# knights-lab/UTree

Hardware: AMD Instinct MI355X
Metric: reads classified/sec, 8 GB L2 CTR, 150 bp reads (higher is better)
Workload: dtype u64; 1 GPU; configs[1]: 1.22e+09-node synthetic L2 CTR (k=32, 21844 labels, image 40.8 GiB, fine_bits=8), 1152000000 x 150 bp reads per GPU (72 steps x 16000000-read batches, 41 distinct batches resident in HBM), RC=0

## Files before the change

utree_amd/csrc/dev_image.c:

```c
#define _FILE_OFFSET_BITS 64
#define _GNU_SOURCE
#define __HIP_PLATFORM_AMD__ 1
#include <hip/hip_runtime_api.h>
#include <fcntl.h>
#include <math.h>
#include <stddef.h>
#include <stdio.h>
#include <stdlib.h>
#include <string.h>
#include <unistd.h>
#include "ctr_host.h"
#include "dev_image.h"

#define HIPCHK(x) do { hipError_t e_ = (x); if (e_ != hipSuccess) { utree_dev_set_hip_error((int)e_, #x); rc = e_ == hipErrorOutOfMemory ? UTREE_E_NOMEM : UTREE_E_HIP; goto fail; } } while (0)
#define KCHK(x) do { int e_ = (x); if (e_ != 0) { utree_dev_set_hip_error(e_, #x); rc = e_ == (int)hipErrorOutOfMemory ? UTREE_E_NOMEM : UTREE_E_HIP; goto fail; } } while (0)

static __thread char g_hip_msg[256];
void utree_dev_set_hip_error(int err, const char *what) {
    snprintf(g_hip_msg, sizeof g_hip_msg, "%s (%d) in %s", hipGetErrorString((hipError_t)err), err, what);
    if (getenv("UTREE_DEBUG")) fprintf(stderr, "[utree_amd] HIP error: %s\n", g_hip_msg);
}
const char *utree_last_hip_error(void) { return g_hip_msg; }
void utree_set_error_text(const char *msg) { snprintf(g_hip_msg, sizeof g_hip_msg, "%s", msg); }

// ... 592 lines not shown
    info->lane_pass = utk_lanes_image_ok(&d->kimg) != 0;
    info->bucket_bytes = 8u * d->hdr.bucket_words;
    info->strand_views = (d->hdr.flags & UTREE_F_STRAND_VIEWS) ? 1u : 0u;
    if (d->hdr.flags & UTREE_F_DIRECT) info->bucket_bytes = 0;
    info->overflow_chains = (d->hdr.flags & UTREE_F_OVF_CHAINS) ? 1u : 0u;
    info->pad0 = 0;
    info->overflow_bytes = (d->hdr.flags & UTREE_F_DIRECT) ? 0 : d->hdr.n_min * d->hdr.rec_words * 8;
    return UTREE_OK;
}

#define LONG_BLOCKS_PER_CU 8

static uint32_t mid_limit(void) {
    static uint32_t v = 0;
    if (!v) {
        const char *e = getenv("UTREE_MID_LIMIT");
        v = UTREE_MID_DEFAULT;
        if (e && atoi(e) >= (int)UTREE_SHORT2_CAP && atoi(e) <= (int)UTREE_MID_CAP) v = (uint32_t)atoi(e);
    }
    return v;
}

static int lanes_enabled(void) { const char *e = getenv("UTREE_LANE_PASS"); return !(e && e[0] == '0'); }

static void ring_lock(utree_dev *d) { while (__atomic_test_and_set(&d->ring_busy, __ATOMIC_ACQUIRE)) ; }
static void ring_unlock(utree_dev *d) { __atomic_clear(&d->ring_busy, __ATOMIC_RELEASE); }

static void ring_collect(utree_dev *d) {
    if (!d->lanes_ring) return;
    ring_lock(d);
    for (unsigned i = 0; i < 64; ++i) {
        const unsigned long long left = d->lanes_ring[2 * i], err = d->lanes_ring[2 * i + 1];
        if (left == ~0ull || err == ~0ull) continue;
        d->lanes_ring[2 * i] = ~0ull; d->lanes_ring[2 * i + 1] = ~0ull;
        d->ring_inflight[i] = 0;
        if (err && !d->dev_error) d->dev_error = err;
        if (timing_on()) fprintf(stderr, "[utree_amd] batch report: %llu of %u reads left by the lane pass, error word %llu\n", left, d->lanes_ring_reads[i], err);
        if (d->lanes_ring_reads[i]) {
            if (left * 4 <= d->lanes_ring_reads[i]) { unsigned long long n = 0, l = 0; for (unsigned w = 0; w < UTREE_LANES_WINDOW; ++w) { n += d->win_reads[w]; l += d->win_left[w]; }
                if (n >= (1u << 18) && l * 4 > n) { memset(d->win_left, 0, sizeof d->win_left); memset(d->win_reads, 0, sizeof d->win_reads); } }
            const unsigned w = d->win_next++ % UTREE_LANES_WINDOW;
            d->win_left[w] = left; d->win_reads[w] = d->lanes_ring_reads[i];
        }
        d->lanes_ring_reads[i] = 0;
    }
    ring_unlock(d);
// ... 63 lines not shown
    char *b = (char *)ws;
    w->cursors = (unsigned long long *)(b + off); off = align_up(off + UTREE_CURSOR_BYTES, 256);
    const uint64_t waves_per_cu = 32 + 20 + 5 * 12;
    w->tally_cap = ((do_rc ? 2 : 1) * total_bases + (uint64_t)n_reads) * 9 / 8 + (uint64_t)d->n_cu * waves_per_cu * UTREE_TALLY_CHUNK + 4096;
    { const char *e = getenv("UTREE_TEST_TALLY_CAP"); if (e && atoll(e) > 0 && (uint64_t)atoll(e) < w->tally_cap) w->tally_cap = (uint64_t)atoll(e); }
    { uint64_t room = w->tally_cap; if (room < UTREE_TALLY_CHUNK) room = UTREE_TALLY_CHUNK; if (room < d->hdr.n_labels) room = d->hdr.n_labels;
      w->tally = (uint64_t *)(b + off); off = align_up(off + room * 8, 256); }
    w->long_list = (uint32_t *)(b + off); off = align_up(off + (uint64_t)n_reads * 4, 256);
    w->mid_list = (uint32_t *)(b + off); off = align_up(off + (uint64_t)n_reads * 4, 256);
    uint64_t max_total = do_rc ? 2 * (uint64_t)max_len + 1 : max_len;
    w->long_blocks = 0; w->hist = NULL; w->touch = NULL;
    w->short_cap = max_total > UTREE_SHORT_CAP ? UTREE_SHORT2_CAP : UTREE_SHORT_CAP;
    w->mid_reads = max_total > w->short_cap;
    w->mid_limit = mid_limit();
    const int lanes_img = utk_lanes_image_ok(&d->kimg);
    if (max_total > w->mid_limit || (lanes_img && max_len > utk_lanes_max_len(&d->kimg))) {
        w->long_blocks = (uint32_t)d->n_cu * LONG_BLOCKS_PER_CU;
        if (w->long_blocks > n_reads) w->long_blocks = n_reads;
        w->hist = (uint32_t *)(b + off); off = align_up(off + (uint64_t)w->long_blocks * d->hdr.n_labels * 4, 256);
        w->touch = (uint32_t *)(b + off); off = align_up(off + (uint64_t)w->long_blocks * ((d->hdr.n_labels + 31) / 32) * 4, 256);
    }
    w->pieces = NULL; w->ltab_rank = w->ltab_cnt = w->lflag = w->long_left = NULL; w->n_long_cap = 0; w->ltally_base = 0;
    w->cls_list = NULL; w->cls_stride = 0; w->n_pieces_cap = 0;
    if (lanes_img && max_len > UTREE_LANES_CAP) {
        w->cls_stride = (n_reads + 63u) & ~63u;
        w->cls_list = (uint32_t *)(b + off); off = align_up(off + (uint64_t)5 * w->cls_stride * 4, 256);
    }
    if (lanes_img && w->long_blocks) {
        uint64_t cap = total_bases / lanes_long_min(d, do_rc) + 1;
        if (cap > n_reads) cap = n_reads;
        const uint64_t piece_windows = 16ull * (UTREE_LANES_CAP - 4 * d->hdr.W + 1);
        const uint64_t n_pieces = total_bases / piece_windows + cap + 1;
        w->n_long_cap = (uint32_t)cap;
        w->n_pieces_cap = n_pieces;
        w->pieces = (uint64_t *)(b + off); off = align_up(off + n_pieces * 8, 256);
        w->ltab_rank = (uint32_t *)(b + off); off = align_up(off + cap * UTREE_LONG_SLOTS * 4, 256);
        w->ltab_cnt = (uint32_t *)(b + off); off = align_up(off + cap * UTREE_LONG_SLOTS * 4, 256);
        w->lflag = (uint32_t *)(b + off); off = align_up(off + cap * 4, 256);
        w->long_left = (uint32_t *)(b + off); off = align_up(off + cap * 4, 256);
        w->ltally_base = (uint64_t)((uint64_t *)(b + off) - w->tally); off = align_up(off + cap * UTREE_LONG_SLOTS * 8, 256);
        { const char *e = getenv("UTREE_TEST_LONG_CAP"); if (e && atoll(e) > 0 && (uint64_t)atoll(e) < w->n_long_cap) w->n_long_cap = (uint32_t)atoll(e); }
        { const char *e = getenv("UTREE_TEST_PIECES_CAP"); if (e && atoll(e) > 0 && (uint64_t)atoll(e) < w->n_pieces_cap) w->n_pieces_cap = (uint64_t)atoll(e); }
    }
    *bytes = (size_t)off;
}

// ... 23 lines not shown
                                 const uint8_t *d_text, uint64_t text_bytes, const uint32_t *d_name_off, const uint32_t *d_name_len) {
    int rc = UTREE_OK;
    if (!d || !d_out || (!d_workspace && n_reads)) return UTREE_E_ARG;
    if (!n_reads) return UTREE_OK;
    if (!d_bases || !d_off || !d_len) return UTREE_E_ARG;
    hipStream_t st = (hipStream_t)stream;
    utk_workspace w; size_t need;
    carve(d, d_workspace, n_reads, total_bases, max_len, do_rc, &w, &need);
    if (workspace_bytes < need) return UTREE_E_ARG;
    HIPCHK(hipSetDevice(d->device));
    HIPCHK(hipMemsetAsync(w.cursors, 0, UTREE_CURSOR_BYTES, st));
    if (w.long_blocks) {
        HIPCHK(hipMemsetAsync(w.hist, 0, (size_t)w.long_blocks * d->hdr.n_labels * 4, st));
        HIPCHK(hipMemsetAsync(w.touch, 0, (size_t)w.long_blocks * ((d->hdr.n_labels + 31) / 32) * 4, st));
    }
    hipEvent_t e0 = NULL, e1 = NULL;
    int tslot = -1;
    if (__atomic_load_n(&d->timing_on, __ATOMIC_ACQUIRE)) {
        tslot = __atomic_fetch_add(&d->n_claimed, 1, __ATOMIC_RELAXED);
        if (tslot >= 0 && tslot < UTREE_MAX_PENDING && 2 * tslot + 1 < d->n_events) { e0 = d->events[2 * tslot]; e1 = d->events[2 * tslot + 1]; }
        else tslot = -1;
    }
    ring_collect(d);
    const int lanes = lanes_enabled() && utk_lanes_image_ok(&d->kimg) && lanes_worth(d);
    if (lanes) {
        const int mixed = max_len > UTREE_LANES_CAP;
        d->last_long = w.long_blocks != 0; d->last_mid = 0; d->last_rc = do_rc; d->last_short_cap = w.short_cap;
        d->last_lanes = utk_lanes_segs(&d->kimg, max_len); d->last_mixed = mixed; d->last_pieces = w.long_blocks != 0;
        if (e0 && !w.long_blocks) HIPCHK(hipEventRecord(e0, st));
        if (!mixed) KCHK(utk_classify_lanes(&d->kimg, d_bases, d_off, d_len, n_reads, max_len, do_rc, d_out, &w, d->n_cu, st));
        else KCHK(utk_classify_lanes_mixed(&d->kimg, d_bases, d_off, d_len, n_reads, max_len, do_rc, d_out, &w, d->n_cu, st));
        if (w.long_blocks) {
            if (e0) HIPCHK(hipEventRecord(e0, st));
            HIPCHK(hipMemsetAsync(w.ltab_rank, 0xFF, (size_t)w.n_long_cap * UTREE_LONG_SLOTS * 4, st));
            HIPCHK(hipMemsetAsync(w.ltab_cnt, 0, (size_t)w.n_long_cap * UTREE_LONG_SLOTS * 4, st));
            HIPCHK(hipMemsetAsync(w.lflag, 0, (size_t)w.n_long_cap * 4, st));
            KCHK(utk_classify_long_pieces(&d->kimg, d_bases, d_off, d_len, do_rc, d_out, &w, d->n_cu, st));
            utk_workspace wl = w;
            wl.long_list = w.long_left;
            wl.long_blocks = w.long_blocks >= 8 ? w.long_blocks / 8 : 1;
            KCHK(utk_classify_long(&d->kimg, d_bases, d_off, d_len, do_rc, d_out, &wl, d->n_cu, st));
            if (e0) { HIPCHK(hipEventRecord(e1, st)); d->recorded[tslot] = 1; }
        }
        KCHK(utk_classify_listed(&d->kimg, d_bases, d_off, d_len, n_reads, max_len, do_rc, d_out, &w, d->n_cu, st));
        if (e0 && !w.long_blocks) { HIPCHK(hipEventRecord(e1, st)); d->recorded[tslot] = 1; }
    } else {
// ... 107 lines not shown
```

utree_amd/csrc/kernels.hip:

```cpp
#include <hip/hip_runtime.h>
#include <stdint.h>
#include <stdio.h>
#include <string.h>
#include "device_common.hpp"
#include "wave_common.hpp"

using namespace utk;

namespace {

#ifdef UTREE_PHASE_TIMERS
__device__ unsigned long long g_phase[16];
struct PhaseT { unsigned long long t, acc[12]; };
#define PH_DECL PhaseT ph_; ph_.t = __builtin_readcyclecounter(); for (int q_ = 0; q_ < 12; ++q_) ph_.acc[q_] = 0;
#define TICKP(ph, i) do { const unsigned long long n_ = __builtin_readcyclecounter(); (ph).acc[i] += n_ - (ph).t; (ph).t = n_; } while (0)
#define TICK(i) TICKP(ph_, i)
#define PH_ARG , PhaseT &ph_
#define PH_PASS , ph_
#define PH_WAITVM asm volatile("s_waitcnt vmcnt(0)" ::: "memory")
#else
#define PH_DECL
#define TICK(i)
#define PH_ARG
#define PH_PASS
// ... 249 lines not shown
        any = any || (nz & low_bytes(total > 4u * g ? total - 4u * g : 0u)) != 0u;
        const uint32_t nib = (nz * 0x00204081u) >> 28;
        const uint32_t nib_next = (uint32_t)__builtin_amdgcn_update_dpp(0, (int)nib, 0x101, 0xF, 0xF, true);
        uint32_t code = g2 ^ ((g2 >> 1) & 0x01010101u);
        code ^= rm & 0x03030303u;
        const uint32_t packed = (code * 0x40100401u) >> 24;
        if (g < ngroups) {
            sb[g ^ 3u] = (uint8_t)packed;
            if (!(lane & 1u)) sbadb[g >> 1] = (uint8_t)(nib | (nib_next << 4));
        }
    }
    return __ballot(any) != 0ull;
}

constexpr int SHORT_CAP = UTREE_SHORT_CAP;
constexpr int SHORT2_CAP = UTREE_SHORT2_CAP;
constexpr int MID_CAP = UTREE_MID_CAP;
constexpr int WAVES_PER_BLOCK = 4;
constexpr uint32_t WORK_GRAB = 32;
constexpr uint32_t TALLY_CHUNK = UTREE_TALLY_CHUNK;
constexpr uint32_t TALLY_DIRECT = UTREE_TALLY_CHUNK / 16;
constexpr int32_t CUT_PENDING = -3;
constexpr int32_t RANK_PENDING = -4;

constexpr int SHORT_MIN_WAVES = 8;
template <int W, int I, bool EXC, typename OFF, int CAP, bool LISTED, int RCMODE = 2>
__global__ __launch_bounds__(256, CAP > SHORT2_CAP ? (I == 2 ? 4 : 3) : (I == 2 ? SHORT_MIN_WAVES : 5))
void classify_short_k(utk_image im, const uint8_t *__restrict__ bases, const uint64_t *__restrict__ off,
                      const uint32_t *__restrict__ len, uint32_t n_reads, int do_rc_arg, utree_result *__restrict__ out,
                      utk_workspace ws) {
    if constexpr (LISTED) { if (!ws.cursors[UTREE_CUR_MID]) return; }
    const int do_rc = RCMODE == 2 ? do_rc_arg : RCMODE;
    constexpr uint32_t K = 4 * W;
    constexpr int NCH = CAP / 64, NWORDS = CAP / 16 + 6;
    __shared__ uint32_t s_words[WAVES_PER_BLOCK][NWORDS + 2];
    __shared__ uint64_t s_bad[WAVES_PER_BLOCK][NCH + 2];
    using HIT = typename std::conditional<I == 2, uint16_t, uint32_t>::type;
    __shared__ HIT s_hits[WAVES_PER_BLOCK][CAP];
    constexpr uint32_t TILE = CAP <= SHORT_CAP ? 256u : KEY_TILE;
    __shared__ uint64_t s_keys[WAVES_PER_BLOCK][TILE + 128];
    __shared__ uint64_t s_reg[256];
    constexpr bool PREFETCH = CAP <= SHORT2_CAP;
    static_assert(PREFETCH || sizeof(HIT) * CAP >= 4 * (RawBuf<CAP>::DW + 4), "raw bytes must fit the hit list");
    __shared__ uint32_t s_raw[PREFETCH ? WAVES_PER_BLOCK : 1][PREFETCH ? RawBuf<CAP>::DW + 4 : 1];
    stage_regions(im, s_reg);
    const RegionLds rg = {s_reg, (uint64_t)(uintptr_t)im.table, im.bucket_words == 16u ? 7u : 6u};
// ... 353 lines not shown
            before = idx ? ((uint32_t)(x1 >> (8 * idx - 8)) & 0xFFu) : prevlast;
            return;
        }
        prevlast = (uint32_t)(x1 >> 56); base += 8;
    }
}

struct VRec { uint64_t w[4]; };
__device__ __forceinline__ VRec vrec(const uint64_t *vt, uint32_t rank) {
    typedef unsigned long long u64x2 __attribute__((ext_vector_type(2)));
    const u64x2 *p = (const u64x2 *)(vt + (size_t)rank * 4);
    const u64x2 a = p[0], b = p[1];
    VRec v; v.w[0] = a.x; v.w[1] = a.y; v.w[2] = b.x; v.w[3] = b.y;
    return v;
}
__device__ __forceinline__ uint32_t v_pid(const VRec &v, uint32_t t) { return (uint32_t)((t < 4 ? v.w[0] : v.w[1]) >> (16u * (t & 3u))) & 0xFFFFu; }
__device__ __forceinline__ uint32_t v_end(const VRec &v, uint32_t t) { return (uint32_t)(v.w[2] >> (8u * t)) & 0xFFu; }
__device__ __forceinline__ bool v_exists(const VRec &v, uint32_t t) { return ((uint32_t)v.w[3] >> t) & 1u; }
__device__ __forceinline__ bool v_more(const VRec &v, uint32_t t) { return ((uint32_t)v.w[3] >> (8u + t)) & 1u; }
__device__ __forceinline__ bool v_us(const VRec &v, uint32_t t) { return ((uint32_t)v.w[3] >> (16u + t)) & 1u; }
__device__ __forceinline__ uint32_t v_len(const VRec &v) { return (uint32_t)(v.w[3] >> 32) & 0xFFu; }
__device__ __forceinline__ uint32_t v_ix(const VRec &v) { return (uint32_t)(v.w[3] >> 48); }

__device__ __forceinline__ void vote_table(const utk_image &im, utree_result *out_r, const uint64_t *T, uint32_t F, uint32_t uix) {
    const uint64_t *vt = im.vote_tab;
    const char *blob = im.label_blob;
    const uint32_t *loff = im.label_off;
    constexpr uint32_t NONE = 0xFFFFFFFFu;
    uint32_t cutoff = cut_of(F);
    uint32_t st = 0, ed = uix, dv = NONE, t = 0, orun = F, sl, ol;
    uint32_t ix_last, n_last, len_last;
    for (;;) {
        const uint64_t t_st = T[st];
        VRec pv = vrec(vt, (uint32_t)t_st);
        const uint64_t t_ed = ed - 1u == st ? t_st : T[ed - 1u];
        const VRec lv = ed - 1u == st ? pv : vrec(vt, (uint32_t)t_ed);
        {
            const uint64_t d0 = pv.w[0] ^ lv.w[0], d1 = pv.w[1] ^ lv.w[1];
            const uint32_t same = d0 ? (uint32_t)__builtin_ctzll(d0) >> 4 : 4u + (d1 ? (uint32_t)__builtin_ctzll(d1) >> 4 : 4u);
            const uint32_t both = ((uint32_t)(pv.w[3] & lv.w[3]) >> 8) & 0xFFu;
            const uint32_t semis = (uint32_t)__builtin_ctz(~both);
            const uint32_t L = same < semis ? same : semis;
            if (L > t) { dv = v_end(pv, L - 1u); t = L; }
        }
        uint32_t run = (uint32_t)(t_st >> 32), td = dv, c1 = run, rp = (uint32_t)t_st;
        bool td_is_end = false;
        bool stopped = false;
        for (uint32_t z = st + 1; z < ed; ++z) {
            const bool is_last = z == ed - 1u;
            const uint64_t tz = is_last ? t_ed : T[z];
            const uint32_t nz = (uint32_t)(tz >> 32), rc = (uint32_t)tz;
            const VRec cv = is_last ? lv : vrec(vt, rc);
            bool aside = false, stop = false;
            if (t >= 8u || !v_exists(pv, t) || (dv == NONE && v_end(pv, 0) == 0u && !v_more(pv, 0))) aside = true;
            else {
                uint32_t a, b, before;
                bool known = true;
                if (v_exists(cv, t) && v_pid(cv, t) == v_pid(pv, t)) {
                    td = v_end(pv, t); td_is_end = true;
                    a = v_more(pv, t) ? ';' : 0u; b = v_more(cv, t) ? ';' : 0u; before = v_us(pv, t) ? '_' : 'x';
                } else if (v_us(pv, t) || !v_exists(cv, t)) {
                    pair_scan(blob + loff[rp], blob + loff[rc], dv + 1u, td, a, b, before);
                    td_is_end = td == v_end(pv, t);
                } else { a = 'a'; b = 'b'; before = 'x'; known = false; }
                if (a == b) run += nz;
                else if ((!a && b == ';') || ((a == ';' || !a) && before == '_')) aside = true;
                else if (run >= cutoff) {
                    ed = z; stop = true;
                    if (!known) {
                        pair_scan(blob + loff[rp], blob + loff[rc], dv + 1u, td, a, b, before);
                        td_is_end = td == v_end(pv, t);
                    }
                } else { run = nz; st = z; }
// ... 5 lines not shown
            }
            if (stop) { stopped = true; break; }
            pv = cv; c1 = nz; rp = rc;
        }
        ix_last = stopped ? v_ix(pv) : v_ix(lv);
        n_last = stopped ? c1 : (uint32_t)(t_ed >> 32);
        len_last = stopped ? v_len(pv) : v_len(lv);
        sl = run; ol = orun;
        if (run < cutoff) break;
        if (st + 1 >= ed) {
            if (n_last >= cutoff) dv = 0xFFFFFFFEu;
            break;
        }
        orun = run; cutoff = cut_of(run);
        if (td != dv) { dv = td; if (td_is_end) ++t; }
    }
    int32_t cut;
    if (dv == NONE) cut = -1;
    else if (dv == 0xFFFFFFFEu) cut = -2;
    else cut = (int32_t)(dv < len_last ? dv : len_last);
    store_result(out_r, ix_last, cut, F, uix, sl, ol);
}

__global__ __launch_bounds__(256) void vote_table_k(utk_image im, utree_result *__restrict__ out, utk_workspace ws, uint32_t n_reads) {
    __shared__ uint32_t s_n[2][4];
    __shared__ uint16_t s_who[256];
    const uint32_t tid = threadIdx.x, wv = tid >> 6, lane = tid & 63u;
    const uint32_t r0 = blockIdx.x * blockDim.x + tid;
    uint32_t cls = 2;
    if (r0 < n_reads) {
        const uint32_t *res = (const uint32_t *)&out[r0];
        const int32_t cut = (int32_t)res[1];
        if (cut == RANK_PENDING) {
            uint32_t *o = (uint32_t *)&out[r0];
            o[0] = im.rank2ix[res[0]]; o[1] = (uint32_t)-2;
        } else if (cut == CUT_PENDING) cls = res[3] == 2u ? 0u : 1u;
    }
    const uint64_t m0 = __builtin_amdgcn_ballot_w64(cls == 0u), m1 = __builtin_amdgcn_ballot_w64(cls == 1u);
    s_who[tid] = 0xFFFFu;
    if (lane == 0) { s_n[0][wv] = (uint32_t)__popcll(m0); s_n[1][wv] = (uint32_t)__popcll(m1); }
    __syncthreads();
    if (cls < 2u) {
        uint32_t before = 0;
        for (uint32_t w = 0; w < wv; ++w) before += s_n[cls][w];
        before += (uint32_t)__popcll((cls ? m1 : m0) & ((1ull << lane) - 1ull));
        s_who[cls ? 255u - before : before] = (uint16_t)tid;
    }
    __syncthreads();
    const uint32_t who = s_who[tid];
    if (who == 0xFFFFu) return;
    const uint32_t r = blockIdx.x * blockDim.x + who;
    const uint32_t *res = (const uint32_t *)&out[r];
    vote_table(im, &out[r], ws.tally + ((uint64_t)res[4] | ((uint64_t)res[5] << 32)), res[2], res[3]);
}

__global__ __launch_bounds__(256) void vote_k(utk_image im, utree_result *__restrict__ out, utk_workspace ws, uint32_t n_reads) {
    const uint32_t r = blockIdx.x * blockDim.x + threadIdx.x;
    if (r >= n_reads) return;
    const uint32_t *res = (const uint32_t *)&out[r];
    if ((int32_t)res[1] == RANK_PENDING) {
        uint32_t *o = (uint32_t *)&out[r];
        o[0] = im.rank2ix[res[0]]; o[1] = (uint32_t)-2;
        return;
    }
    if ((int32_t)res[1] != CUT_PENDING) return;
    const uint32_t F = res[2], uix = res[3];
    const uint64_t *T = ws.tally + ((uint64_t)res[4] | ((uint64_t)res[5] << 32));
    const char *blob = im.label_blob;
    const uint32_t *loff = im.label_off;
    uint32_t cutoff = cut_of(F);
    uint32_t st = 0, ed = uix, dv = 0xFFFFFFFFu, orun = F, sl, ol;
    for (;;) {
        const uint64_t t_st = T[st];
        {
            const char *sa = blob + loff[(uint32_t)t_st], *sz = blob + loff[(uint32_t)T[ed - 1]];
            uint32_t base = dv + (dv == 0xFFFFFFFFu), q = 0xFFFFFFFFu;
            bool first = dv != 0xFFFFFFFFu;
            for (;;) {
                uint64_t a[2], b[2];
                label16(sa, base, a[0], a[1]); label16(sz, base, b[0], b[1]);
                bool stop = false;
#pragma unroll
                for (int h = 0; h < 2; ++h) {
                    const uint64_t x = a[h], d = a[h] ^ b[h], sx = a[h] ^ 0x3B3B3B3B3B3B3B3Bull;
                    uint64_t end = ((x - 0x0101010101010101ull) & ~x) & 0x8080808080808080ull;
                    end |= (((d & 0x7F7F7F7F7F7F7F7Full) + 0x7F7F7F7F7F7F7F7Full) | d) & 0x8080808080808080ull;
                    uint64_t semi = ~(((sx & 0x7F7F7F7F7F7F7F7Full) + 0x7F7F7F7F7F7F7F7Full) | sx) & 0x8080808080808080ull;
                    if (h == 0 && first) { end &= ~0xFFull; semi &= ~0xFFull; }
                    if (end) semi &= (end & (0ull - end)) - 1ull;
                    if (semi) q = base + 8u * (uint32_t)h + ((63u - (uint32_t)__builtin_clzll(semi)) >> 3);
                    if (end) { stop = true; break; }
                }
                if (stop) break;
                base += 16; first = false;
            }
            if (q != 0xFFFFFFFFu) dv = q;
        }
        uint32_t run = (uint32_t)(t_st >> 32), td = dv;
        const char *s1 = blob + loff[(uint32_t)t_st];
        uint32_t c1 = run;
        const uint32_t probe = dv + (dv == 0xFFFFFFFFu);
        const bool skip0 = dv != 0xFFFFFFFFu;
        uint64_t x1_first, y1_first;
        label16(s1, probe, x1_first, y1_first);
        for (uint32_t z = st + 1; z < ed; ++z) {
            const uint64_t tz = T[z];
            const uint32_t nz = (uint32_t)(tz >> 32);
            const char *s2 = blob + loff[(uint32_t)tz];
            uint64_t x1 = x1_first, y1 = y1_first;
            uint64_t x2_first, y2_first;
            label16(s2, probe, x2_first, y2_first);
            bool aside = false, stop = false;
            if (!(x1 & 0xFFull)) aside = true;
            else {
                uint64_t x2 = x2_first, y2 = y2_first;
                uint32_t base = probe, idx, prevlast = 0;
                bool first = true;
                for (;;) {
                    uint64_t m = stop_flags(x1, x2);
                    if (first && skip0) m &= ~0xFFull;
                    if (m) { idx = (uint32_t)(__builtin_ctzll(m) >> 3); break; }
                    prevlast = (uint32_t)(x1 >> 56);
                    base += 8; first = false;
                    m = stop_flags(y1, y2);
                    x1 = y1; x2 = y2;
                    if (m) { idx = (uint32_t)(__builtin_ctzll(m) >> 3); break; }
                    prevlast = (uint32_t)(x1 >> 56);
                    base += 8;
                    label16(s1, base, x1, y1); label16(s2, base, x2, y2);
                }
                td = base + idx;
                const uint32_t a = (uint32_t)(x1 >> (8 * idx)) & 0xFFu, b = (uint32_t)(x2 >> (8 * idx)) & 0xFFu;
                const uint32_t before = idx ? ((uint32_t)(x1 >> (8 * idx - 8)) & 0xFFu) : (first ? 0u : prevlast);
                if (a == b) run += nz;
                else if ((!a && b == ';') || ((a == ';' || !a) && before == '_')) aside = true;
                else if (run >= cutoff) { ed = z; stop = true; }
                else { run = nz; st = z; }
            }
            if (aside) {
                run = nz; st = z;
                orun -= c1;
                cutoff = cut_of(orun);
            }
            if (stop) break;
            s1 = s2; c1 = nz; x1_first = x2_first; y1_first = y2_first;
        }
        sl = run; ol = orun;
        if (run < cutoff) break;
        if (st + 1 >= ed) {
            if ((uint32_t)(T[ed - 1] >> 32) >= cutoff) dv = 0xFFFFFFFEu;
            break;
        }
        orun = run; dv = td; cutoff = cut_of(run);
    }
    const uint32_t rk = (uint32_t)T[ed - 1];
    int32_t cut;
    if (dv == 0xFFFFFFFFu) cut = -1;
    else if (dv == 0xFFFFFFFEu) cut = -2;
    else { uint32_t Ls = loff[rk + 1] - loff[rk] - 1; cut = (int32_t)(dv < Ls ? dv : Ls); }
    store_result(&out[r], im.rank2ix[rk], cut, F, uix, sl, ol);
}

template <int W, int I, bool EXC, typename OFF>
__global__ void lookup_k(utk_image im, const uint64_t *__restrict__ hi, const uint64_t *__restrict__ lo, uint64_t n,
                         uint32_t *__restrict__ ix) {
    for (uint64_t i = (uint64_t)blockIdx.x * blockDim.x + threadIdx.x; i < n; i += (uint64_t)gridDim.x * blockDim.x) {
        uint32_t rank = lookup_word<W, I, EXC, OFF>(im, W == 16 ? hi[i] : 0ull, lo[i]);
        ix[i] = rank == INVALID ? INVALID : im.rank2ix[rank];
    }
}

constexpr uint32_t MODEL_CAP = 640;
template <int W, int I>
__global__ __launch_bounds__(256) void model_k(utk_image im, const uint8_t *__restrict__ bases, const uint64_t *__restrict__ off,
                                               const uint32_t *__restrict__ len, uint32_t n_reads, int do_rc,
                                               unsigned long long *__restrict__ counts) {
    constexpr uint32_t K = 4 * W;
    __shared__ uint64_t s_b[4][MODEL_CAP];
    const uint32_t lane = lane_id(), wv = threadIdx.x >> 6;
    unsigned long long c_reads = 0, c_win = 0, c_buck = 0, c_line = 0, c_over = 0;
    for (uint32_t r = blockIdx.x * 4 + wv; r < n_reads; r += gridDim.x * 4) {
        const uint32_t L = len[r];
        const uint64_t o = off[r];
// ... 179 lines not shown
```

utree_amd/csrc/lanes_core.hpp:

```cpp
#pragma once
#include <hip/hip_runtime.h>
#include <stdint.h>
#include <stdio.h>
#include <string.h>
#include "device_common.hpp"
#include "wave_common.hpp"

using namespace utk;

namespace {

#ifdef UTREE_LANES_TIMERS
__device__ unsigned long long g_lphase[8];
#define LT_DECL unsigned long long lt_t = __builtin_readcyclecounter(), lt_acc[6] = {0, 0, 0, 0, 0, 0};
#define LT(i) do { const unsigned long long n_ = __builtin_readcyclecounter(); lt_acc[i] += n_ - lt_t; lt_t = n_; } while (0)
#else
#define LT_DECL
#define LT(i)
#endif

constexpr int LANES_WAVES = 4;
constexpr int LANES_WPS = 3;
constexpr uint32_t LCAP = UTREE_LANES_CAP;
constexpr uint32_t NWORD = LCAP / 16;
static_assert(LCAP % 32 == 0, "slot geometry");
static_assert(LCAP + 16 + 48 <= 256, "positions are 8-bit fields of a run record");
template <int W> struct Geo {
    static constexpr uint32_t K = 4 * W, OFS = UTREE_MIN_MARGIN(W), NB = K - 15 - 2 * OFS;
    static constexpr uint32_t NA = W == 16 ? 3 : 1;
    static constexpr uint32_t FRONT = NA;
    static constexpr uint32_t STRIDE = NWORD + FRONT + 2;
    static constexpr uint32_t RUNS = W == 16 ? 512 : 1280;
    static constexpr uint32_t DNONE = 63;
    static_assert((STRIDE & 1) == 1, "slot geometry");
};
constexpr uint32_t TSLOTS = 12;
constexpr uint32_t T_EMPTY = 0xFFFFFFFFu;
constexpr int32_t CUT_PENDING = -3, RANK_PENDING = -4;

__device__ __forceinline__ uint32_t low_bytes(uint32_t n) { return n >= 4u ? 0xFFFFFFFFu : ((1u << (8u * n)) - 1u); }
__device__ __forceinline__ uint64_t ballot64(bool p) { return __builtin_amdgcn_ballot_w64(p); }
__device__ __forceinline__ uint32_t umin(uint32_t a, uint32_t b) { return a < b ? a : b; }
__device__ __forceinline__ uint32_t wave_max_u32(uint32_t v) { return ~wave_min_u32(~v); }

__device__ __forceinline__ void store_result(utree_result *out, uint32_t label, int32_t cut, uint32_t found, uint32_t uix, uint32_t sl, uint32_t ol) {
    uint32_t *o = (uint32_t *)out;
    o[0] = label; o[1] = (uint32_t)cut; o[2] = found; o[3] = uix; o[4] = sl; o[5] = ol;
}

typedef const __attribute__((address_space(1))) uint32_t *gptr32;


__device__ __forceinline__ void rest96(const uint32_t (&A)[3], const uint32_t (&B)[3], uint32_t pos, uint32_t &r0, uint32_t &r1, uint32_t &r2) {
    const uint32_t sh = 2u * pos, bs = sh & 31u;
    const bool w1 = (sh & 32u) != 0u, w2 = (sh & 64u) != 0u;
    const uint32_t v[6] = {A[0], A[1], A[2], B[0], B[1], B[2]};
    uint32_t y[6];
#pragma unroll
    for (int t = 0; t < 6; ++t) y[t] = w1 ? (t ? v[t - 1] : 0u) : v[t];
    uint32_t x[4];
#pragma unroll
// ... 658 lines not shown
                    }
                }
            }
            wave_lds_fence();
            LT(4);
            continue;
        }
        const uint64_t xm = ballot64(have && exc);
        if (xm) {
            unsigned long long xb = 0;
            if (lane == 0) xb = atomicAdd(&ws.cursors[UTREE_CUR_MID], (unsigned long long)__popcll(xm));
            xb = uni64(xb);
            if (have && exc) ws.mid_list[xb + lanes_below(xm)] = r;
        }
        const bool live = have && !exc;
        const uint32_t *tq = tab + (lane < RPW ? lane : 0u);
        uint32_t nu = 0, F = 0;
        if (live) {
#pragma unroll
            for (uint32_t i = 0; i < TSR; ++i) { const uint32_t e = tq[i * RPW]; if (e != T_EMPTY) { ++nu; F += e & CMASK; } }
        }
        const uint32_t first_rank = tq[0] >> CB;
        const uint32_t maxnu = uni32(wave_max_u32(nu));
        const uint32_t need = nu >= 2u ? nu : 0u;
        uint32_t incl = need;
#pragma unroll
        for (int dd = 1; dd < 64; dd <<= 1) { const uint32_t t = __shfl_up(incl, dd); if (lane >= (uint32_t)dd) incl += t; }
        const uint32_t total = uni32((uint32_t)__shfl(incl, 63));
        if (total > chunk_left) {
            unsigned long long nb = 0;
            if (lane == 0) {
                nb = atomicAdd(&ws.cursors[0], (unsigned long long)UTREE_TALLY_CHUNK);
                if (nb + UTREE_TALLY_CHUNK > ws.tally_cap) { ws.cursors[UTREE_CUR_ERROR] = UTREE_DEVERR_TALLY_CAP; nb = 0; }
            }
            chunk_base = uni64(nb);
            chunk_left = UTREE_TALLY_CHUNK;
        }
        const unsigned long long my_base = chunk_base + (incl - need);
        chunk_base += total; chunk_left -= total;
        if (maxnu >= 2u) {
            for (uint32_t i = 0; i < maxnu; ++i) {
                const uint32_t e = tq[i * RPW];
                uint32_t place = 0;
                for (uint32_t j = 0; j < maxnu; ++j) { const uint32_t x = tq[j * RPW]; place += (j < nu && (x >> CB) < (e >> CB)) ? 1u : 0u; }
                if (need && i < nu) ws.tally[my_base + place] = (uint64_t)(e >> CB) | ((uint64_t)(e & CMASK) << 32);
            }
        }
        if (live) {
            if (F == 0) store_result(&out[r], 0, -2, 0, 0, 0, 0);
            else if (nu == 1) store_result(&out[r], first_rank, RANK_PENDING, F, 1, 0, 0);
            else store_result(&out[r], 0, CUT_PENDING, F, nu, (uint32_t)my_base, (uint32_t)(my_base >> 32));
        }
        wave_lds_fence();
        LT(4);
    }
#ifdef UTREE_LANES_TIMERS
    if (lane == 0) { for (int q = 0; q < 6; ++q) atomicAdd(&g_lphase[q], lt_acc[q]); atomicAdd(&g_lphase[7], 1ull); }
#endif
}

#define LANES_PROLOGUE(W_) \
    using G_ = Geo<W_>; \
    __shared__ uint32_t s_stream[LANES_WAVES][64 * G_::STRIDE]; \
    __shared__ uint32_t s_runs[LANES_WAVES][G_::RUNS]; \
    __shared__ uint32_t s_tab[LANES_WAVES][64 * TSLOTS]; \
    __shared__ uint32_t s_full[LANES_WAVES][2]; \
    __shared__ uint32_t s_pref[LANES_WAVES][64]; \
    __shared__ uint64_t s_ost[LANES_WAVES][64]; \
    __shared__ uint64_t s_reg[256]; \
    for (uint32_t x = threadIdx.x; x < 256; x += blockDim.x) s_reg[x] = im.regions[x]; \
    const uint32_t wv = uni32(threadIdx.x >> 6); \
    { uint32_t *sl_ = s_stream[wv] + lane_id() * G_::STRIDE + G_::FRONT; \
      _Pragma("unroll") for (uint32_t i = 1; i <= G_::FRONT; ++i) sl_[-(int)i] = 0;       \
// ... 52 lines not shown
```

utree_amd/csrc/lanes_kernel.hip:

```cpp
#include <hip/hip_runtime.h>
#include <stdint.h>
#include <stdio.h>
#include <stdlib.h>
#include <string.h>
#include "device_common.hpp"
#include "wave_common.hpp"

using namespace utk;

extern "C" {
#define PART_DECL(W_, I_, NL_, BS_) int utk_lanes_part_##W_##_##I_##_##NL_##_##BS_(int segs, int irr, int mode, const utk_image *im, const uint8_t *d_bases, const uint64_t *d_off, \
                                                                              const uint32_t *d_len, uint32_t n_reads, int do_rc, utree_result *d_out, const utk_workspace *ws, \
                                                                              int n_cu, void *stream, uint32_t cls);
PART_DECL(8, 2, 1, 0) PART_DECL(8, 2, 1, 1) PART_DECL(8, 2, 2, 0) PART_DECL(8, 4, 1, 0) PART_DECL(8, 4, 1, 1) PART_DECL(8, 4, 2, 0)
PART_DECL(16, 2, 1, 0) PART_DECL(16, 2, 1, 1) PART_DECL(16, 2, 2, 0)
#undef PART_DECL
}

namespace {

constexpr uint32_t LCAP = UTREE_LANES_CAP;
constexpr int32_t CUT_PENDING = -3, RANK_PENDING = -4;
__device__ __forceinline__ uint64_t ballot64(bool p) { return __builtin_amdgcn_ballot_w64(p); }
__device__ __forceinline__ void store_result(utree_result *out, uint32_t label, int32_t cut, uint32_t found, uint32_t uix, uint32_t sl, uint32_t ol) {
    uint32_t *o = (uint32_t *)out;
    o[0] = label; o[1] = (uint32_t)cut; o[2] = found; o[3] = uix; o[4] = sl; o[5] = ol;
}

}

extern "C" int utk_lanes_both_strands(const utk_image *im, int do_rc) {
    const char *e = getenv("UTREE_LANES_BS");
    return do_rc && im->bucket_words == 8u && (im->flags & UTREE_F_STRAND_VIEWS) && !(e && atoi(e) == 0);
}

namespace {

int lanes_launch(const utk_image *im, int segs, int mode, const uint8_t *d_bases, const uint64_t *d_off, const uint32_t *d_len, uint32_t n_reads, int do_rc,
                 utree_result *d_out, const utk_workspace *ws, int n_cu, void *stream, uint32_t cls) {
    const int irr = im->irr_n != 0, nl = im->bucket_words == 16u ? 2 : 1;
    const int bs = utk_lanes_both_strands(im, do_rc);
#define PART(W_, I_, NL_, BS_) return utk_lanes_part_##W_##_##I_##_##NL_##_##BS_(segs, irr, mode, im, d_bases, d_off, d_len, n_reads, do_rc, d_out, ws, n_cu, stream, cls)
    if (im->W == 16) { if (nl == 2) PART(16, 2, 2, 0); if (bs) PART(16, 2, 1, 1); PART(16, 2, 1, 0); }
    if (im->I == 4) { if (nl == 2) PART(8, 4, 2, 0); if (bs) PART(8, 4, 1, 1); PART(8, 4, 1, 0); }
    if (nl == 2) PART(8, 2, 2, 0);
// ... 166 lines not shown
```

utree_amd/csrc/utree_internal.h:

```cpp
#ifndef UTREE_INTERNAL_H
#define UTREE_INTERNAL_H
#include <stddef.h>
#include <stdint.h>
#include <stdlib.h>
#include <time.h>
#include "../../include/utree_amd.h"

#ifdef __cplusplus
extern "C" {
#endif

#define UTREE_NUMBINS ((1u << 24) + 1u)
#define UTREE_INVALID 0xFFFFFFFFu
#define UTREE_IMG_MAGIC 0x31474d4945525455ull
#define UTREE_IMG_HEADER_BYTES 4096u
#define UTREE_IMG_VERSION 14u
#define UTREE_REGION_NB_BITS 25
#define UTREE_REGION_SUB_BITS 9
#define UTREE_REGION_BASE_SHIFT (UTREE_REGION_NB_BITS + UTREE_REGION_SUB_BITS)
#define UTREE_MIN_MARGIN(W_) ((W_) == 16 ? 2u : 0u)
#define UTREE_TALLY_CHUNK 8192u
#define UTREE_CUR_LONG 32
#define UTREE_CUR_MID 16
#define UTREE_CUR_WORK 48
// ... 84 lines not shown
                       void *d_out, void *stream);
int utk_fill_recs_pad(uint64_t *d_recs_end, uint32_t words, void *stream);

typedef struct {
    unsigned long long *cursors;
    uint64_t *tally;
    uint64_t tally_cap;
    uint32_t *long_list;
    uint32_t *mid_list;
    uint32_t *hist;
    uint32_t *touch;
    uint32_t long_blocks, mid_reads;
    uint32_t short_cap;
    uint32_t mid_limit;
    uint64_t *pieces;
    uint32_t *ltab_rank, *ltab_cnt;
    uint32_t *lflag;
    uint32_t *long_left;
    uint32_t n_long_cap;
    uint64_t n_pieces_cap;
    uint32_t *cls_list;
    uint32_t cls_stride;
    uint64_t ltally_base;
} utk_workspace;

int utk_classify_short(const utk_image *im, const uint8_t *d_bases, const uint64_t *d_off, const uint32_t *d_len,
                       uint32_t n_reads, int do_rc, utree_result *d_out, const utk_workspace *ws, int n_cu,
                       void *stream);
int utk_lanes_ok(const utk_image *im, uint32_t max_len, int do_rc);
int utk_lanes_segs(const utk_image *im, uint32_t max_len);
int utk_lanes_image_ok(const utk_image *im);
int utk_lanes_both_strands(const utk_image *im, int do_rc);
int utk_classify_long_pieces(const utk_image *im, const uint8_t *d_bases, const uint64_t *d_off, const uint32_t *d_len, int do_rc,
                             utree_result *d_out, const utk_workspace *ws, int n_cu, void *stream);
int utk_classify_lanes(const utk_image *im, const uint8_t *d_bases, const uint64_t *d_off, const uint32_t *d_len, uint32_t n_reads,
                       uint32_t max_len, int do_rc, utree_result *d_out, const utk_workspace *ws, int n_cu, void *stream);
int utk_classify_lanes_mixed(const utk_image *im, const uint8_t *d_bases, const uint64_t *d_off, const uint32_t *d_len, uint32_t n_reads,
                             uint32_t max_len, int do_rc, utree_result *d_out, const utk_workspace *ws, int n_cu, void *stream);
uint32_t utk_lanes_max_len(const utk_image *im);
int utk_route(const uint32_t *d_len, uint32_t n_reads, int do_rc, const utk_workspace *ws, void *stream);
int utk_classify_mid(const utk_image *im, const uint8_t *d_bases, const uint64_t *d_off, const uint32_t *d_len,
                     uint32_t n_reads, int do_rc, utree_result *d_out, const utk_workspace *ws, int n_cu, void *stream);
int utk_classify_listed(const utk_image *im, const uint8_t *d_bases, const uint64_t *d_off, const uint32_t *d_len,
                        uint32_t n_reads, uint32_t max_len, int do_rc, utree_result *d_out, const utk_workspace *ws, int n_cu, void *stream);
int utk_classify_long(const utk_image *im, const uint8_t *d_bases, const uint64_t *d_off, const uint32_t *d_len,
                      int do_rc, utree_result *d_out, const utk_workspace *ws, int n_cu, void *stream);
// ... 40 lines not shown
```

Measured before the change: 2.327 billion reads/s.

## Pack two- and three-entry tallies inline in result record, skip tally buffer

Reads with two or three distinct label ranks now store their sorted packed (rank,count) entries directly in the result record under a new CUT_INLINE marker, instead of reserving space in the global tally buffer. The vote kernels read entries through a TallyList accessor that decodes either form, and vote_table_k gains a third class so the 3-entry inline reads are grouped separately. The change is meant to cut tally-chunk atomics, prefix-scan work and scattered global writes and reads for the common small-tally case. It also sets launch bounds occupancy to 6 on vote_table_k, and it relies on counts and ranks fitting in the packed bit widths.

```diff
diff --git a/utree_amd/csrc/dev_image.c b/utree_amd/csrc/dev_image.c
--- a/utree_amd/csrc/dev_image.c
+++ b/utree_amd/csrc/dev_image.c
@@ -638,6 +638,7 @@
 }
 
 static int lanes_enabled(void) { const char *e = getenv("UTREE_LANE_PASS"); return !(e && e[0] == '0'); }
+static int tally_inline_enabled(void) { const char *e = getenv("UTREE_TALLY_INLINE"); return !(e && e[0] == '0'); }
 
 static void ring_lock(utree_dev *d) { while (__atomic_test_and_set(&d->ring_busy, __ATOMIC_ACQUIRE)) ; }
 static void ring_unlock(utree_dev *d) { __atomic_clear(&d->ring_busy, __ATOMIC_RELEASE); }
@@ -747,6 +748,7 @@
     }
     w->pieces = NULL; w->ltab_rank = w->ltab_cnt = w->lflag = w->long_left = NULL; w->n_long_cap = 0; w->ltally_base = 0;
     w->cls_list = NULL; w->cls_stride = 0; w->n_pieces_cap = 0;
+    w->tally_inline = 0;
     if (lanes_img && max_len > UTREE_LANES_CAP) {
         w->cls_stride = (n_reads + 63u) & ~63u;
         w->cls_list = (uint32_t *)(b + off); off = align_up(off + (uint64_t)5 * w->cls_stride * 4, 256);
@@ -816,6 +818,7 @@
         else tslot = -1;
     }
     ring_collect(d);
+    w.tally_inline = !rd && !srd && tally_inline_enabled();
     const int lanes = lanes_enabled() && utk_lanes_image_ok(&d->kimg) && lanes_worth(d);
     if (lanes) {
         const int mixed = max_len > UTREE_LANES_CAP;
diff --git a/utree_amd/csrc/kernels.hip b/utree_amd/csrc/kernels.hip
--- a/utree_amd/csrc/kernels.hip
+++ b/utree_amd/csrc/kernels.hip
@@ -295,6 +295,7 @@
 constexpr uint32_t TALLY_DIRECT = UTREE_TALLY_CHUNK / 16;
 constexpr int32_t CUT_PENDING = -3;
 constexpr int32_t RANK_PENDING = -4;
+constexpr int32_t CUT_INLINE = -5;
 
 constexpr int SHORT_MIN_WAVES = 8;
 template <int W, int I, bool EXC, typename OFF, int CAP, bool LISTED, int RCMODE = 2>
@@ -694,7 +695,23 @@
 __device__ __forceinline__ uint32_t v_len(const VRec &v) { return (uint32_t)(v.w[3] >> 32) & 0xFFu; }
 __device__ __forceinline__ uint32_t v_ix(const VRec &v) { return (uint32_t)(v.w[3] >> 48); }
 
-__device__ __forceinline__ void vote_table(const utk_image &im, utree_result *out_r, const uint64_t *T, uint32_t F, uint32_t uix) {
+struct TallyList {
+    const uint64_t *tally;
+    uint32_t a, b, c, cb;
+    bool packed;
+    __device__ __forceinline__ uint64_t entry(uint32_t i) const {
+        if (packed) {
+            const uint32_t w = i == 0u ? a : i == 1u ? b : c;
+            return (uint64_t)(w >> cb) | ((uint64_t)(w & ((1u << cb) - 1u)) << 32);
+        }
+        return tally[((uint64_t)b | ((uint64_t)c << 32)) + i];
+    }
+};
+__device__ __forceinline__ TallyList tally_list(const utk_image &im, const utk_workspace &ws, const uint32_t *res) {
+    return TallyList{ws.tally, res[0], res[4], res[5], im.I == 4u ? 13u : 16u, (int32_t)res[1] == CUT_INLINE};
+}
+
+__device__ __forceinline__ void vote_table(const utk_image &im, utree_result *out_r, const TallyList &T, uint32_t F, uint32_t uix) {
     const uint64_t *vt = im.vote_tab;
     const char *blob = im.label_blob;
     const uint32_t *loff = im.label_off;
@@ -703,9 +720,9 @@
     uint32_t st = 0, ed = uix, dv = NONE, t = 0, orun = F, sl, ol;
     uint32_t ix_last, n_last, len_last;
     for (;;) {
-        const uint64_t t_st = T[st];
+        const uint64_t t_st = T.entry(st);
         VRec pv = vrec(vt, (uint32_t)t_st);
-        const uint64_t t_ed = ed - 1u == st ? t_st : T[ed - 1u];
+        const uint64_t t_ed = ed - 1u == st ? t_st : T.entry(ed - 1u);
         const VRec lv = ed - 1u == st ? pv : vrec(vt, (uint32_t)t_ed);
         {
             const uint64_t d0 = pv.w[0] ^ lv.w[0], d1 = pv.w[1] ^ lv.w[1];
@@ -720,7 +737,7 @@
         bool stopped = false;
         for (uint32_t z = st + 1; z < ed; ++z) {
             const bool is_last = z == ed - 1u;
-            const uint64_t tz = is_last ? t_ed : T[z];
+            const uint64_t tz = is_last ? t_ed : T.entry(z);
             const uint32_t nz = (uint32_t)(tz >> 32), rc = (uint32_t)tz;
             const VRec cv = is_last ? lv : vrec(vt, rc);
             bool aside = false, stop = false;
@@ -772,58 +789,51 @@
     store_result(out_r, ix_last, cut, F, uix, sl, ol);
 }
 
-__global__ __launch_bounds__(256) void vote_table_k(utk_image im, utree_result *__restrict__ out, utk_workspace ws, uint32_t n_reads) {
-    __shared__ uint32_t s_n[2][4];
+__global__ __launch_bounds__(256, 6) void vote_table_k(utk_image im, utree_result *__restrict__ out, utk_workspace ws, uint32_t n_reads) {
+    constexpr uint32_t NC = 3;
+    __shared__ uint32_t s_n[NC][4];
     __shared__ uint16_t s_who[256];
     const uint32_t tid = threadIdx.x, wv = tid >> 6, lane = tid & 63u;
     const uint32_t r0 = blockIdx.x * blockDim.x + tid;
-    uint32_t cls = 2;
+    uint32_t cls = NC;
     if (r0 < n_reads) {
         const uint32_t *res = (const uint32_t *)&out[r0];
         const int32_t cut = (int32_t)res[1];
         if (cut == RANK_PENDING) {
             uint32_t *o = (uint32_t *)&out[r0];
             o[0] = im.rank2ix[res[0]]; o[1] = (uint32_t)-2;
-        } else if (cut == CUT_PENDING) cls = res[3] == 2u ? 0u : 1u;
-    }
-    const uint64_t m0 = __builtin_amdgcn_ballot_w64(cls == 0u), m1 = __builtin_amdgcn_ballot_w64(cls == 1u);
+        } else if (cut == CUT_PENDING || cut == CUT_INLINE) cls = res[3] == 2u ? 0u : res[3] == 3u ? 1u : 2u;
+    }
+    const uint64_t m0 = __builtin_amdgcn_ballot_w64(cls == 0u), m1 = __builtin_amdgcn_ballot_w64(cls == 1u), m2 = __builtin_amdgcn_ballot_w64(cls == 2u);
     s_who[tid] = 0xFFFFu;
-    if (lane == 0) { s_n[0][wv] = (uint32_t)__popcll(m0); s_n[1][wv] = (uint32_t)__popcll(m1); }
+    if (lane == 0) { s_n[0][wv] = (uint32_t)__popcll(m0); s_n[1][wv] = (uint32_t)__popcll(m1); s_n[2][wv] = (uint32_t)__popcll(m2); }
     __syncthreads();
-    if (cls < 2u) {
+    if (cls < NC) {
         uint32_t before = 0;
         for (uint32_t w = 0; w < wv; ++w) before += s_n[cls][w];
-        before += (uint32_t)__popcll((cls ? m1 : m0) & ((1ull << lane) - 1ull));
-        s_who[cls ? 255u - before : before] = (uint16_t)tid;
+        const uint64_t mine = cls == 0u ? m0 : cls == 1u ? m1 : m2;
+        before += (uint32_t)__popcll(mine & ((1ull << lane) - 1ull));
+        if (cls == 1u) before += s_n[0][0] + s_n[0][1] + s_n[0][2] + s_n[0][3];
+        s_who[cls == 2u ? 255u - before : before] = (uint16_t)tid;
     }
     __syncthreads();
     const uint32_t who = s_who[tid];
     if (who == 0xFFFFu) return;
     const uint32_t r = blockIdx.x * blockDim.x + who;
     const uint32_t *res = (const uint32_t *)&out[r];
-    vote_table(im, &out[r], ws.tally + ((uint64_t)res[4] | ((uint64_t)res[5] << 32)), res[2], res[3]);
-}
-
-__global__ __launch_bounds__(256) void vote_k(utk_image im, utree_result *__restrict__ out, utk_workspace ws, uint32_t n_reads) {
-    const uint32_t r = blockIdx.x * blockDim.x + threadIdx.x;
-    if (r >= n_reads) return;
-    const uint32_t *res = (const uint32_t *)&out[r];
-    if ((int32_t)res[1] == RANK_PENDING) {
-        uint32_t *o = (uint32_t *)&out[r];
-        o[0] = im.rank2ix[res[0]]; o[1] = (uint32_t)-2;
-        return;
-    }
-    if ((int32_t)res[1] != CUT_PENDING) return;
     const uint32_t F = res[2], uix = res[3];
-    const uint64_t *T = ws.tally + ((uint64_t)res[4] | ((uint64_t)res[5] << 32));
+    vote_table(im, &out[r], tally_list(im, ws, res), F, uix);
+}
+
+__device__ __forceinline__ void vote_bytes(const utk_image &im, utree_result *out_r, const TallyList &T, uint32_t F, uint32_t uix) {
     const char *blob = im.label_blob;
     const uint32_t *loff = im.label_off;
     uint32_t cutoff = cut_of(F);
     uint32_t st = 0, ed = uix, dv = 0xFFFFFFFFu, orun = F, sl, ol;
     for (;;) {
-        const uint64_t t_st = T[st];
+        const uint64_t t_st = T.entry(st);
         {
-            const char *sa = blob + loff[(uint32_t)t_st], *sz = blob + loff[(uint32_t)T[ed - 1]];
+            const char *sa = blob + loff[(uint32_t)t_st], *sz = blob + loff[(uint32_t)T.entry(ed - 1u)];
             uint32_t base = dv + (dv == 0xFFFFFFFFu), q = 0xFFFFFFFFu;
             bool first = dv != 0xFFFFFFFFu;
             for (;;) {
@@ -854,7 +864,7 @@
         uint64_t x1_first, y1_first;
         label16(s1, probe, x1_first, y1_first);
         for (uint32_t z = st + 1; z < ed; ++z) {
-            const uint64_t tz = T[z];
+            const uint64_t tz = T.entry(z);
             const uint32_t nz = (uint32_t)(tz >> 32);
             const char *s2 = blob + loff[(uint32_t)tz];
             uint64_t x1 = x1_first, y1 = y1_first;
@@ -898,17 +908,32 @@
         sl = run; ol = orun;
         if (run < cutoff) break;
         if (st + 1 >= ed) {
-            if ((uint32_t)(T[ed - 1] >> 32) >= cutoff) dv = 0xFFFFFFFEu;
+            if ((uint32_t)(T.entry(ed - 1u) >> 32) >= cutoff) dv = 0xFFFFFFFEu;
             break;
         }
         orun = run; dv = td; cutoff = cut_of(run);
     }
-    const uint32_t rk = (uint32_t)T[ed - 1];
+    const uint32_t rk = (uint32_t)T.entry(ed - 1u);
     int32_t cut;
     if (dv == 0xFFFFFFFFu) cut = -1;
     else if (dv == 0xFFFFFFFEu) cut = -2;
     else { uint32_t Ls = loff[rk + 1] - loff[rk] - 1; cut = (int32_t)(dv < Ls ? dv : Ls); }
-    store_result(&out[r], im.rank2ix[rk], cut, F, uix, sl, ol);
+    store_result(out_r, im.rank2ix[rk], cut, F, uix, sl, ol);
+}
+
+__global__ __launch_bounds__(256) void vote_k(utk_image im, utree_result *__restrict__ out, utk_workspace ws, uint32_t n_reads) {
+    const uint32_t r = blockIdx.x * blockDim.x + threadIdx.x;
+    if (r >= n_reads) return;
+    const uint32_t *res = (const uint32_t *)&out[r];
+    const int32_t pend = (int32_t)res[1];
+    if (pend == RANK_PENDING) {
+        uint32_t *o = (uint32_t *)&out[r];
+        o[0] = im.rank2ix[res[0]]; o[1] = (uint32_t)-2;
+        return;
+    }
+    if (pend != CUT_PENDING && pend != CUT_INLINE) return;
+    const uint32_t F = res[2], uix = res[3];
+    vote_bytes(im, &out[r], tally_list(im, ws, res), F, uix);
 }
 
 template <int W, int I, bool EXC, typename OFF>
diff --git a/utree_amd/csrc/lanes_core.hpp b/utree_amd/csrc/lanes_core.hpp
--- a/utree_amd/csrc/lanes_core.hpp
+++ b/utree_amd/csrc/lanes_core.hpp
@@ -37,6 +37,7 @@
 constexpr uint32_t TSLOTS = 12;
 constexpr uint32_t T_EMPTY = 0xFFFFFFFFu;
 constexpr int32_t CUT_PENDING = -3, RANK_PENDING = -4;
+constexpr int32_t CUT_INLINE = -5;
 
 __device__ __forceinline__ uint32_t low_bytes(uint32_t n) { return n >= 4u ? 0xFFFFFFFFu : ((1u << (8u * n)) - 1u); }
 __device__ __forceinline__ uint64_t ballot64(bool p) { return __builtin_amdgcn_ballot_w64(p); }
@@ -741,23 +742,25 @@
         }
         const uint32_t first_rank = tq[0] >> CB;
         const uint32_t maxnu = uni32(wave_max_u32(nu));
-        const uint32_t need = nu >= 2u ? nu : 0u;
-        uint32_t incl = need;
-#pragma unroll
-        for (int dd = 1; dd < 64; dd <<= 1) { const uint32_t t = __shfl_up(incl, dd); if (lane >= (uint32_t)dd) incl += t; }
-        const uint32_t total = uni32((uint32_t)__shfl(incl, 63));
-        if (total > chunk_left) {
-            unsigned long long nb = 0;
-            if (lane == 0) {
-                nb = atomicAdd(&ws.cursors[0], (unsigned long long)UTREE_TALLY_CHUNK);
-                if (nb + UTREE_TALLY_CHUNK > ws.tally_cap) { ws.cursors[UTREE_CUR_ERROR] = UTREE_DEVERR_TALLY_CAP; nb = 0; }
-            }
-            chunk_base = uni64(nb);
-            chunk_left = UTREE_TALLY_CHUNK;
-        }
-        const unsigned long long my_base = chunk_base + (incl - need);
-        chunk_base += total; chunk_left -= total;
-        if (maxnu >= 2u) {
+        const bool inl = ws.tally_inline != 0u;
+        const uint32_t need = nu >= (inl ? 4u : 2u) ? nu : 0u;
+        unsigned long long my_base = 0;
+        if (ballot64(need != 0u)) {
+            uint32_t incl = need;
+#pragma unroll
+            for (int dd = 1; dd < 64; dd <<= 1) { const uint32_t t = __shfl_up(incl, dd); if (lane >= (uint32_t)dd) incl += t; }
+            const uint32_t total = uni32((uint32_t)__shfl(incl, 63));
+            if (total > chunk_left) {
+                unsigned long long nb = 0;
+                if (lane == 0) {
+                    nb = atomicAdd(&ws.cursors[0], (unsigned long long)UTREE_TALLY_CHUNK);
+                    if (nb + UTREE_TALLY_CHUNK > ws.tally_cap) { ws.cursors[UTREE_CUR_ERROR] = UTREE_DEVERR_TALLY_CAP; nb = 0; }
+                }
+                chunk_base = uni64(nb);
+                chunk_left = UTREE_TALLY_CHUNK;
+            }
+            my_base = chunk_base + (incl - need);
+            chunk_base += total; chunk_left -= total;
             for (uint32_t i = 0; i < maxnu; ++i) {
                 const uint32_t e = tq[i * RPW];
                 uint32_t place = 0;
@@ -768,6 +771,11 @@
         if (live) {
             if (F == 0) store_result(&out[r], 0, -2, 0, 0, 0, 0);
             else if (nu == 1) store_result(&out[r], first_rank, RANK_PENDING, F, 1, 0, 0);
+            else if (!need) {
+                const uint32_t e0 = tq[0], e1 = tq[RPW], e2 = tq[2u * RPW];
+                const uint32_t lo = umin(e0, e1), hi = e0 ^ e1 ^ lo, m = umin(hi, e2);
+                store_result(&out[r], umin(lo, m), CUT_INLINE, F, nu, lo ^ m ^ umin(lo, m), hi ^ e2 ^ m);
+            }
             else store_result(&out[r], 0, CUT_PENDING, F, nu, (uint32_t)my_base, (uint32_t)(my_base >> 32));
         }
         wave_lds_fence();
diff --git a/utree_amd/csrc/lanes_kernel.hip b/utree_amd/csrc/lanes_kernel.hip
--- a/utree_amd/csrc/lanes_kernel.hip
+++ b/utree_amd/csrc/lanes_kernel.hip
@@ -21,6 +21,7 @@
 
 constexpr uint32_t LCAP = UTREE_LANES_CAP;
 constexpr int32_t CUT_PENDING = -3, RANK_PENDING = -4;
+[[maybe_unused]] constexpr int32_t CUT_INLINE = -5;
 __device__ __forceinline__ uint64_t ballot64(bool p) { return __builtin_amdgcn_ballot_w64(p); }
 __device__ __forceinline__ void store_result(utree_result *out, uint32_t label, int32_t cut, uint32_t found, uint32_t uix, uint32_t sl, uint32_t ol) {
     uint32_t *o = (uint32_t *)out;
diff --git a/utree_amd/csrc/utree_internal.h b/utree_amd/csrc/utree_internal.h
--- a/utree_amd/csrc/utree_internal.h
+++ b/utree_amd/csrc/utree_internal.h
@@ -130,6 +130,7 @@
     uint32_t *cls_list;
     uint32_t cls_stride;
     uint64_t ltally_base;
+    uint32_t tally_inline;
 } utk_workspace;
 
 int utk_classify_short(const utk_image *im, const uint8_t *d_bases, const uint64_t *d_off, const uint32_t *d_len,
```

Measured after the change: 2.406 billion reads/s (median of 6 runs). 1.03x the previous value.
